# 51616/split-vae

Measured on AMD Instinct MI355X. Metric: images/sec training step, SPLIT-VAE CelebA-64 bs512, higher is better.
Workload: dtype f32 operands, f32 accumulate (exact-fp32 MFMA v_mfma_f32_16x16x4_f32): the reference's precision (vae/model.py:12); 1 GPU; SPLIT-VAE CelebA-64 64x64 beta=120 patch_size=8 latents=128+128 lr=1e-4, full train step (scramble+fwd+ELBO+bwd+Adam), per-GPU batch 512; global_batch=512, per_gpu_batch=512, parallelism=dp1, reconstructions=not stored (dead after the fused loss)

## Files before the change

split_vae_amd/csrc/kernels.h:

```cpp
#pragma once
#include <hip/hip_runtime.h>
#include <stdint.h>

#define SV_MAX_TAPS 81

struct TapGemmArgs {
  const void* A;
  const void* Wt;
  const float* bias;
  void* out;
  const void* mask;
  int M;
  int lOY, lOX;
  int OY, OX;
  int IH, IW, lda;
  int cl2;
  int P;
  int Ktot;
  int S, SX;
  int N;
  int OHF, OWF, OS, ooy, oox, ldo;
  int act, out_f32, splitk, ntaps;
  int ups;
  int d2s;
  int d2s_y;
  int clampin;
  int s2d3;
  const float* nll_img; void* nll_grad; float* nll_part; int nll_ch; float nll_gscale;
  int nll_noout;
  const float* fix;
  const float* fix2; int fix_nc, fix_pad;
  int cls_n;
  int accum;
  int adj;
  int8_t dy[SV_MAX_TAPS];
  int8_t dx[SV_MAX_TAPS];
};
int svk_tap_gemm(const TapGemmArgs& a, int dtype, int cfg, hipStream_t st);
#define SV_TAP_MAX_MULTI 4
struct TapGemmMulti {
  TapGemmArgs a[SV_TAP_MAX_MULTI];
  int zbase[SV_TAP_MAX_MULTI];
  int n;
};
int svk_tap_gemm_multi(const TapGemmArgs* a, int n, int dtype, int cfg, hipStream_t st);

struct TileConvArgs {
  const void* A; const void* Wt; const float* bias; void* out; const void* mask;
  int B, IH, IW, lda;
  int cl2, P, Ktot, S, SX;
  int lTW, lTH, lNB;
  int OY, OX, tilesX, tilesY, ntiles;
  int TIW, TIH, y_lo, x_lo;
  int PS;
  int plane_bytes;
  int nph, lnph;
  int xcd_chunk;
  int off_bytes, in_bytes;
  int buf_bytes;
  int wslots;
  int N, OHF, OWF, OS, ooy, oox, ldo, act, out_f32, ntaps;
  int dbg;
  int ups;
  int d2s;
  int cls_n;
  int d2s_y, clampin;
  int s2d3;
  int dma;
  const float* fix;
  const float* fix2; int fix_nc, fix_pad;
  const float* nll_img; void* nll_grad; float* nll_part; int nll_ch; float nll_gscale; int nll_noout;
  int8_t dy[SV_MAX_TAPS];
  int8_t dx[SV_MAX_TAPS];
};
#define SV_MAX_MULTI 8
#define SV_SHARED_STREAMS 3
hipStream_t sv_shared_stream(int k);
struct TileConvMulti { TileConvArgs a[SV_MAX_MULTI]; };
bool svk_tile_conv_plan(const TapGemmArgs& t, int dtype, int B, TileConvArgs* a, int* cfg_out);
int svk_tile_conv_multi(const TileConvArgs* a, int n, int dtype, int cfg, hipStream_t st);
int svk_conv_dispatch_multi(const TapGemmArgs* t, int n, int dtype, int tap_cfg, hipStream_t st);
int svk_tile_conv(const TileConvArgs& a, int dtype, int cfg, hipStream_t st);
int svk_row_conv_try(const TapGemmArgs* t, int n, int dtype, hipStream_t st);
bool svk_row_conv_supported(const TapGemmArgs* t, int n, int dtype);
int svk_conv_dispatch(const TapGemmArgs& t, int dtype, int tap_cfg, hipStream_t st);

struct WgradArgs {
  const void* A;
  const void* dY;
  float* dW;
  float* dbias;
  int M, lOY, lOX, OY, OX, IH, IW, lda, S, SX;
  int fold_kw, fold_c;
  int ldy, ycols;
  int cl2;
  int Cin_pad, Cin_real, N, Nrows;
  int ntaps, msplit;
  int ups;
  int clampin;
  int dy_s2d;
  int dy_os, dy_oy, dy_ox;
  int assign;
  int s2d3;
  float* ws;
  int64_t ws_bytes;
  hipEvent_t ev_mid[2];
  struct WgradReduceDesc* defer; int* n_defer;
  int8_t dy[SV_MAX_TAPS];
  int8_t dx[SV_MAX_TAPS];
};
int svk_wgrad(const WgradArgs& a, int dtype, int cfg, hipStream_t st);
#define SV_WGRAD_IM2COL_MAX_MULTI 4
struct WgradMulti {
  WgradArgs a[SV_WGRAD_IM2COL_MAX_MULTI];
  int zbase[SV_WGRAD_IM2COL_MAX_MULTI];
  int plain[SV_WGRAD_IM2COL_MAX_MULTI];
  int n;
};
int svk_wgrad_multi(const WgradArgs* a, int n, int dtype, int cfg, hipStream_t st);

struct WgradTileArgs {
  const void* A; const void* dY; float* dW; float* dbias;
  float* slab; float* ws; int64_t ws_bytes;
  float* bslab;
  struct WgradReduceDesc* defer; int* n_defer;
  int B, IH, IW, lda, cl2, S, SX, fold_kw, fold_c;
  int layer_id;
  int contig;
  int pairx;
  int lTW, lTH, lNB, OY, OX, tilesX, tilesY, ntiles;
  int TIW, TIH, y_lo, x_lo, PS;
  int ldy, YS, lycp;
// ... 126 lines not shown
```

split_vae_amd/csrc/lgvae_plan.hip:

```cpp
#include <string>
#include <algorithm>
#include <vector>
#include <map>
#include <stdio.h>
#include <stdlib.h>
#include <string.h>
#include "common.hip.h"
#include "kernels.h"
#include "conv_geom.h"

namespace {

__global__ void sv_plan_spin_kernel(long long ticks) {
  const long long t0 = wall_clock64();
  while (wall_clock64() - t0 < ticks) __builtin_amdgcn_s_sleep(32);
}
static void sv_plan_spin(hipStream_t st, int us) { hipLaunchKernelGGL(sv_plan_spin_kernel, dim3(1), dim3(64), 0, st, (long long)us * 100); }

struct Buf { std::string name; int64_t off, bytes; };

struct ParamInfo { std::string name; int64_t off; int ndim; int64_t shape[4]; int64_t count; };

static std::vector<ParamInfo> build_params(const sv_lgvae_desc* d) {
  std::vector<ParamInfo> v;
// ... 137 lines not shown
  int early_wait(hipStream_t st) {
    if (!early_pending) return SV_OK;
    early_pending = false;
    return hipStreamWaitEvent(st, ev_early_now, 0) == hipSuccess ? SV_OK : (int)hipGetLastError();
  }
  bool ensure_side() {
    if (nside) return true;
    {
      static const int want = getenv("SV_SIDE_STREAMS") ? atoi(getenv("SV_SIDE_STREAMS")) : 2;
      const int k = want < 1 ? 1 : want > SIDE_MAX - 1 ? SIDE_MAX - 1 : want;
      if (!ev_fork && hipEventCreateWithFlags(&ev_fork, hipEventDisableTiming) != hipSuccess) return false;
      for (int i = 0; i < k && i < SV_SHARED_STREAMS; ++i) {
        side[i] = sv_shared_stream(i);
        if (!side[i]) break;
        (void)hipEventCreateWithFlags(&ev_join[i], hipEventDisableTiming);
        ++nside;
      }
    }
    return nside > 0;
  }
  hipStream_t wgrad_stream(hipStream_t st) {
    side_slot = 0;
    if (!side_allowed()) return st;
    if (!ensure_side()) return st;
    const int use = side_use < nside ? side_use : nside;
    static const char* order = getenv("SV_SIDE_ORDER");
    int slot = side_next % use;
    if (order && order[0]) { const int c = order[side_count % (int)strlen(order)] - '0'; if (c >= 0 && c < use) slot = c; }
    ++side_count;
    hipEvent_t ef = fresh_event(ev_fork);
    if (hipEventRecord(ef, st) != hipSuccess || hipStreamWaitEvent(side[slot], ef, 0) != hipSuccess) return st;
    side_used[slot] = true;
    if (dbg_side_delay_us > 0 && side_count == 1) sv_plan_spin(side[slot], dbg_side_delay_us);
    side_next = slot + 1;
    side_slot = slot;
    side_pending = true;
    return side[slot];
  }
  int join_side(hipStream_t st) {
    const bool cap = graph_on || dyn;
    if (!side_pending && !(cap && side_used[0])) return SV_OK;
    side_pending = false;
    side_next = 0;
    side_count = 0;
    for (int i = 0; i < nside; ++i) {
      if (cap && !side_used[i]) continue;
      hipEvent_t ej = fresh_event(ev_join[i]);
      if (hipEventRecord(ej, side[i]) != hipSuccess || hipStreamWaitEvent(st, ej, 0) != hipSuccess) return (int)hipGetLastError();
    }
    return SV_OK;
  }
  int dbg_side_delay_us = 0;
  bool dbg_bucket_skip_side = false;
  hipEvent_t ev_bucket[3][1 + SIDE_MAX] = {};
  bool bucket_rec[3][1 + SIDE_MAX] = {};
  bool buckets_now = false;
  void clear_buckets() {
    for (auto& row : bucket_rec)
      for (auto& b : row) b = false;
  }
  int record_bucket(int k, hipStream_t st) {
    for (int i = 0; i <= SIDE_MAX; ++i) bucket_rec[k][i] = false;
    for (int i = 0; i <= nside; ++i) {
      hipStream_t s = i == 0 ? st : side[i - 1];
      if (i > 0 && !s) continue;
      if (!ev_bucket[k][i] && hipEventCreateWithFlags(&ev_bucket[k][i], hipEventDisableTiming) != hipSuccess) return (int)hipGetLastError();
      if (hipEventRecord(ev_bucket[k][i], s) != hipSuccess) return (int)hipGetLastError();
      bucket_rec[k][i] = true;
    }
    return SV_OK;
  }
  bool graph_on = false;
  const SvDynArgs* dyn = nullptr;
  struct HostState { bool gz_clean, dz_slabs, dz_valid, gz_zero_skipped, nll_fused; };
  HostState host_state() const { return {gz_clean, dz_slabs, dz_valid, gz_zero_skipped, nll_fused}; }
  void set_host_state(const HostState& h) { gz_clean = h.gz_clean; dz_slabs = h.dz_slabs; dz_valid = h.dz_valid; gz_zero_skipped = h.gz_zero_skipped; nll_fused = h.nll_fused; }
  uint64_t host_state_bits() const { return (uint64_t)gz_clean | (uint64_t)dz_slabs << 1 | (uint64_t)dz_valid << 2 | (uint64_t)gz_zero_skipped << 3 | (uint64_t)nll_fused << 4; }
  struct GraphEntry { hipGraphExec_t exec = nullptr; int seen = 0; HostState exit_state{}; };
  std::map<std::vector<uint64_t>, GraphEntry> graphs;
  bool prof_on;
  std::string prof_filter;
  std::vector<ProfEntry> prof;
  std::map<std::string, int> profidx;
  std::vector<ProfPending> pending;
  std::vector<hipEvent_t> event_pool;

  size_t esz() const { return d.dtype == SV_BF16 ? 2 : 4; }
  int ndec() const { return d.global_only ? 1 : 2; }
  int lc() const { return d.global_only ? d.global_latent : d.global_latent + d.local_latent; }
  int64_t add_buf(const std::string& n, int64_t bytes) {
    Buf b;
    b.name = n; b.off = ws_bytes; b.bytes = bytes;
    ws_bytes += (bytes + 255) / 256 * 256;
    bufidx[n] = (int)bufs.size();
    bufs.push_back(b);
    return b.off;
  }
  void* bp(const std::string& n) const {
    auto it = bufidx.find(n);
    return it == bufidx.end() ? nullptr : (void*)(ws + bufs[it->second].off);
  }
  int64_t bbytes(const std::string& n) const { return bufs[bufidx.at(n)].bytes; }
};

namespace {

// ... 1057 lines not shown
  build_buffers(p);
  *out = p;
  return SV_OK;
}

extern "C" void sv_lgvae_plan_destroy(sv_lgvae_plan* p) {
  if (!p) return;
  for (auto& pe : p->pending) { (void)hipEventDestroy(pe.a); (void)hipEventDestroy(pe.b); }
  for (auto e : p->event_pool) (void)hipEventDestroy(e);
  for (int i = 0; i < p->nside; ++i) {
    (void)hipStreamSynchronize(p->side[i]);
    (void)hipEventDestroy(p->ev_join[i]);
  }
  if (p->ev_fork) (void)hipEventDestroy(p->ev_fork);
  if (p->ev_early) (void)hipEventDestroy(p->ev_early);
  for (auto e : p->ev_cap)
    if (e) (void)hipEventDestroy(e);
  for (auto& row : p->ev_bucket)
    for (auto e : row)
      if (e) (void)hipEventDestroy(e);
  if (!p->graphs.empty()) (void)hipDeviceSynchronize();
  for (auto& kv : p->graphs)
    if (kv.second.exec) (void)hipGraphExecDestroy(kv.second.exec);
  delete p;
}

extern "C" int64_t sv_lgvae_workspace_bytes(const sv_lgvae_plan* p) { return p ? p->ws_bytes : -1; }

extern "C" int sv_lgvae_plan_bind(sv_lgvae_plan* p, void* workspace, int64_t bytes, void* stream) {
  if (!p || !workspace) return SV_E_BADARG;
  if (bytes < p->ws_bytes) return SV_E_WORKSPACE;
  if ((uintptr_t)workspace & 255) return SV_E_BADARG;
  p->ws = (char*)workspace;
  hipStream_t st = (hipStream_t)stream;
  hipError_t e = hipMemsetAsync(workspace, 0, (size_t)p->ws_bytes, st);
  if (e != hipSuccess) return (int)e;
  e = hipMemcpyAsync(p->bp("jobs"), p->jobs.data(), p->jobs.size() * sizeof(PrepJob), hipMemcpyHostToDevice, st);
  if (e != hipSuccess) return (int)e;
  e = hipStreamSynchronize(st);
  if (e != hipSuccess) return (int)e;
  p->bound = true;
  return SV_OK;
}

extern "C" int sv_lgvae_buffer(const sv_lgvae_plan* p, const char* name, int64_t* offset, int64_t* bytes) {
  if (!p || !name) return SV_E_BADARG;
  auto it = p->bufidx.find(name);
  if (it == p->bufidx.end()) return SV_E_BADARG;
  if (offset) *offset = p->bufs[it->second].off;
  if (bytes) *bytes = p->bufs[it->second].bytes;
  return SV_OK;
}

static int run_phases(sv_lgvae_plan* p, const sv_lgvae_step_args* s, hipStream_t st) {
  const int ph = s->phases;
  p->n_cap = 0;
  for (auto& u : p->side_used) u = false;
  {
    static const int forced = getenv("SV_SIDE_STREAMS") ? atoi(getenv("SV_SIDE_STREAMS")) : 0;
    const bool whole = (ph & SV_PHASE_ALL) == SV_PHASE_ALL;
    p->side_use = forced > 0 ? forced : (whole && p->ndec() * p->d.B >= 512) ? 2 : 1;
  }
  const bool zero_here = (ph & SV_PHASE_LOSS) && s->grads;
  hipStream_t early = ((ph & SV_PHASE_PREP) && (ph & SV_PHASE_FWD_ENCODERS)) ? p->early_stream(st) : nullptr;
  if (early && zero_here) {
    if (hipMemsetAsync(s->grads, 0, (size_t)p->nparams * 4, early) != hipSuccess) return (int)hipGetLastError();
  }
  if (ph & SV_PHASE_PREP) SV_TRY(phase_prep(p, s, st, early));
  if (early) SV_TRY(p->early_done(early));
  static const bool no_fused_nll = getenv("SV_NO_FUSED_NLL") != nullptr;
  static const bool no_fused_nll_f32 = getenv("SV_NO_FUSED_NLL_F32") != nullptr;
  const bool want_nll = !no_fused_nll && (ph & SV_PHASE_FWD_DECODERS) && (ph & SV_PHASE_LOSS) && s->grads && s->images6 &&
                        (p->d.dtype == SV_BF16 || !no_fused_nll_f32);
  if (!(ph & SV_PHASE_FORWARD)) p->nll_fused = false;
  if (ph & SV_PHASE_FORWARD) SV_TRY(phase_forward(p, s, ph & SV_PHASE_FWD_ENCODERS, ph & SV_PHASE_FWD_DECODERS, st, want_nll));
  if (ph & SV_PHASE_LOSS) {
    if (s->grads && !early) {
      Scope sc(p, st, "zero_grads", 0, (double)p->nparams * 4);
      if (hipMemsetAsync(s->grads, 0, (size_t)p->nparams * 4, st) != hipSuccess) return (int)hipGetLastError();
    }
    SV_TRY(phase_loss(p, s, s->grads != nullptr, st));
  }
  SV_TRY(p->early_wait(st));
  const bool buckets = (ph & SV_PHASE_BUCKET_EVENTS) && !p->graph_on && !p->dyn;
  if (ph & SV_PHASE_BACKWARD) p->clear_buckets();
  p->buckets_now = buckets;
  if (ph & SV_PHASE_BWD_DECODERS) {
    SV_TRY(phase_bwd_decoders(p, s, st));
    if (buckets) SV_TRY(p->record_bucket(0, st));
  }
  if (ph & (SV_PHASE_BWD_ENC_HEADS | SV_PHASE_BWD_ENC_CONVS))
    SV_TRY(phase_bwd_encoders(p, s, ph & SV_PHASE_BWD_ENC_HEADS, ph & SV_PHASE_BWD_ENC_CONVS, st, buckets));
  SV_TRY(p->join_side(st));
  if (p->n_pending) {
    Scope sc(p, st, "wgrad.all.reduce", 0, 0);
    const int np = p->n_pending;
    p->n_pending = 0;
    SV_TRY(svk_wgrad_reduce_all(p->red_pending, np, st));
  }
  if (ph & SV_PHASE_ADAM) {
    Scope sc(p, st, "adam_step", 0, (double)p->nparams * 28);
    SV_TRY(svk_adam_step(s->params, s->grads, s->adam_m, s->adam_v, p->nparams, s->lr, s->beta1, s->beta2,
                         s->adam_eps, s->t, s->grad_scale, p->dyn, st));
  }
  return SV_OK;
}

// ... 25 lines not shown
  const float alpha = (ph & SV_PHASE_ADAM) ? (float)svk_adam_alpha(s->lr, s->beta1, s->beta2, s->t) : 0.f;
  SV_TRY(svk_set_dyn((SvDynArgs*)p->bp("dyn"), s->seed, s->step, s->sample_offset, alpha, st));
  if (!e.exec) {
    hipGraph_t g = nullptr;
    if (hipStreamBeginCapture(st, hipStreamCaptureModeThreadLocal) != hipSuccess) return (int)hipGetLastError();
    p->dyn = (const SvDynArgs*)p->bp("dyn");
    const int rc = run_phases(p, s, st);
    p->dyn = nullptr;
    const hipError_t he = hipStreamEndCapture(st, &g);
    if (rc || he != hipSuccess || !g) {
      if (g) (void)hipGraphDestroy(g);
      return rc ? rc : (int)he;
    }
    const hipError_t hi = hipGraphInstantiate(&e.exec, g, nullptr, nullptr, 0);
    (void)hipGraphDestroy(g);
    if (hi != hipSuccess) { e.exec = nullptr; return (int)hi; }
    e.exit_state = p->host_state();
  } else {
    p->set_host_state(e.exit_state);
  }
  if (hipGraphLaunch(e.exec, st) != hipSuccess) return (int)hipGetLastError();
  return SV_OK;
}

extern "C" int sv_lgvae_graph_enable(sv_lgvae_plan* p, int32_t enable) {
  if (!p) return SV_E_BADARG;
  if (enable && p->d.global_only) return SV_E_UNSUPPORTED;
  p->graph_on = enable != 0;
  if (!enable) {
    for (auto& kv : p->graphs)
      if (kv.second.exec) (void)hipGraphExecDestroy(kv.second.exec);
    p->graphs.clear();
  }
  return SV_OK;
}

extern "C" int sv_lgvae_bucket_wait(sv_lgvae_plan* p, int32_t bucket, void* stream) {
  if (!p || bucket < 0 || bucket > 3) return SV_E_BADARG;
  int n = 0;
  for (int k = (bucket == 3 ? 1 : bucket); k <= (bucket == 3 ? 2 : bucket); ++k)
    for (int i = 0; i <= sv_lgvae_plan::SIDE_MAX; ++i)
      if (p->bucket_rec[k][i]) {
        if (p->dbg_bucket_skip_side && i > 0) continue;
        if (hipStreamWaitEvent((hipStream_t)stream, p->ev_bucket[k][i], 0) != hipSuccess) return (int)hipGetLastError();
        ++n;
      }
  return n ? SV_OK : SV_E_STATE;
}

extern "C" int sv_lgvae_plan_debug(sv_lgvae_plan* p, const char* key, int64_t value) {
  if (!p || !key) return SV_E_BADARG;
  if (!strcmp(key, "side_delay_us")) { if (value < 0 || value > 1000000) return SV_E_BADARG; p->dbg_side_delay_us = (int)value; return SV_OK; }
  if (!strcmp(key, "bucket_skip_side")) { p->dbg_bucket_skip_side = value != 0; return SV_OK; }
  return SV_E_BADARG;
}

extern "C" int sv_lgvae_graph_count(const sv_lgvae_plan* p) {
  if (!p) return SV_E_BADARG;
  int n = 0;
  for (auto& kv : p->graphs) n += kv.second.exec != nullptr;
  return n;
}

extern "C" int sv_lgvae_profile_enable(sv_lgvae_plan* p, int32_t enable) {
  if (!p) return SV_E_BADARG;
  p->prof_on = enable != 0;
  if (enable) {
    for (auto& pe : p->pending) { p->event_pool.push_back(pe.a); p->event_pool.push_back(pe.b); }
    p->pending.clear();
    p->prof.clear();
    p->profidx.clear();
  }
  return SV_OK;
}

extern "C" int sv_lgvae_profile_filter(sv_lgvae_plan* p, const char* name) {
  if (!p) return SV_E_BADARG;
  p->prof_filter = name ? name : "";
  return SV_OK;
}

extern "C" int sv_lgvae_profile_read(sv_lgvae_plan* p, int32_t max_entries, char names[][64], double* total_ms,
                                     int32_t* launches, double* flops_per_launch, double* bytes_per_launch) {
  if (!p) return SV_E_BADARG;
  for (auto& pe : p->pending) {
    (void)hipEventSynchronize(pe.b);
    float ms = 0.f;
    if (hipEventElapsedTime(&ms, pe.a, pe.b) == hipSuccess) {
      p->prof[pe.entry].total_ms += ms;
      p->prof[pe.entry].launches += 1;
    }
    p->event_pool.push_back(pe.a);
    p->event_pool.push_back(pe.b);
  }
  p->pending.clear();
  int n = (int)p->prof.size();
  if (n > max_entries) n = max_entries;
  for (int i = 0; i < n; ++i) {
    if (names) snprintf(names[i], 64, "%s", p->prof[i].name.c_str());
    if (total_ms) total_ms[i] = p->prof[i].total_ms;
    if (launches) launches[i] = p->prof[i].launches;
    if (flops_per_launch) flops_per_launch[i] = p->prof[i].flops;
    if (bytes_per_launch) bytes_per_launch[i] = p->prof[i].bytes;
  }
  return n;
}
// ... 19 lines not shown
```

split_vae_amd/csrc/tile_conv.hip:

```cpp
#include "common.hip.h"
#include "kernels.h"
#include "tile_stage.hip.h"
#include "dlogistic.hip.h"
#include <stdio.h>
#include <stdlib.h>
#include <string.h>

#ifndef SV_TC_PPS16
#define SV_TC_PPS16 16
#endif
#ifndef SV_TC_PPS32
#define SV_TC_PPS32 8
#endif
#ifndef SV_TC_PPS64
#define SV_TC_PPS64 8
#endif
static __host__ __device__ constexpr int tile_pps(int BN, int YR = 0) {
  return YR ? (BN == 16 || YR == 5 ? YR * 4 : 8) : BN == 16 ? SV_TC_PPS16 : BN == 32 ? SV_TC_PPS32 : BN == 64 ? SV_TC_PPS64 : 8;
}

template <int PPS>
__device__ __forceinline__ int wpiece(int q, int n) {
  if constexpr (PPS % 8 == 0) return q ^ (n & 7);
  else return (q & ~7) == (PPS & ~7) ? (q & ~3) | ((q & 3) ^ (n & 3)) : q ^ (n & 7);
}

template <typename T> struct MmaOpT;
template <> struct MmaOpT<bf16_t> {
  static __device__ __forceinline__ void run(const uint4& a, const uint4& b, f32x4& c) {
    c = __builtin_amdgcn_mfma_f32_16x16x32_bf16(__builtin_bit_cast(bf16x8, a), __builtin_bit_cast(bf16x8, b), c, 0, 0, 0);
  }
};
template <> struct MmaOpT<float> {
  static __device__ __forceinline__ void run(const uint4& a, const uint4& b, f32x4& c) {
    const float4 af = __builtin_bit_cast(float4, a), bf = __builtin_bit_cast(float4, b);
    c = __builtin_amdgcn_mfma_f32_16x16x4f32(af.x, bf.x, c, 0, 0, 0);
    c = __builtin_amdgcn_mfma_f32_16x16x4f32(af.y, bf.y, c, 0, 0, 0);
    c = __builtin_amdgcn_mfma_f32_16x16x4f32(af.z, bf.z, c, 0, 0, 0);
    c = __builtin_amdgcn_mfma_f32_16x16x4f32(af.w, bf.w, c, 0, 0, 0);
  }
};

static constexpr int tile_min_waves(int BN, int NW, int YR, bool WR = false) { return (YR || WR) && NW == 4 ? (BN == 64 ? 3 : 4) : 1; }
template <typename T, int BN, int MF, int NW, int YR, bool WR, bool FX = false>
__global__ __launch_bounds__(64 * NW, tile_min_waves(BN, NW, YR, WR)) void tile_conv_kernel(const TileConvMulti mg) {
  const TileConvArgs& g = mg.a[blockIdx.z];
  if (SV_DBG(g.dbg) & 32) return;
  constexpr int NT = 64 * NW, WM = 16 * MF, BM = NW * WM, NF = BN / 16;
  constexpr int PPS = tile_pps(BN, YR), RB = PPS * 16;
  constexpr int RPP = NT / PPS;
  constexpr int BRN = (BN + RPP - 1) / RPP;
  constexpr int EPP = ElemTraits<T>::EPP;
  extern __shared__ __attribute__((aligned(16))) char smem[];
  char* sB = smem;
  int* sOff = (int*)(smem + g.wslots * BN * RB);
  char* sIn = smem + g.wslots * BN * RB + g.off_bytes;

  const int tid = threadIdx.x, lane = tid & 63, wave = tid >> 6;
  int t = blockIdx.x;
  if (g.xcd_chunk) {
    const int remapped = (t & 7) * g.xcd_chunk + (t >> 3);
    t = remapped < g.ntiles && (g.ntiles & 7) == 0 ? remapped : t;
  }
  const int tx0 = (t % g.tilesX) << g.lTW; t /= g.tilesX;
  const int ty0 = (t % g.tilesY) << g.lTH; t /= g.tilesY;
  const int b0 = t << g.lNB;
  const int n0 = blockIdx.y * BN;
  const int TW = 1 << g.lTW, TH = 1 << g.lTH, NB = 1 << g.lNB;
  const int cpp = 1 << g.cl2;

  const T* __restrict__ Wb = (const T*)g.Wt;
  const int nph = g.nph, lcH = g.cl2 - g.lnph;
  const int gP = g.P >> g.lnph, gKtot = g.Ktot, gdbg = SV_DBG(g.dbg);
  const int pp = tid % PPS, r0 = tid / PPS;
  int ph = 0;
  uint4 rbA[BRN];
  auto load_b = [&](int ks, uint4 (&rb)[BRN]) {
    const int pl = ks * PPS + pp;
    const bool pv = pl < gP;
    const int p = ((pl >> lcH) << g.cl2) + (ph << lcH) + (pl & ((1 << lcH) - 1));
#pragma unroll
    for (int i = 0; i < BRN; ++i) {
      const int n = r0 + RPP * i;
      rb[i] = (pv && n < BN && r0 < RPP) ? *(const uint4*)(Wb + (int64_t)(n0 + n) * gKtot + (int64_t)p * EPP) : make_uint4(0, 0, 0, 0);
    }
  };
  auto write_b = [&](int slot, const uint4 (&rb)[BRN]) {
#pragma unroll
    for (int i = 0; i < BRN; ++i) {
      const int n = r0 + RPP * i;
      if (n < BN && r0 < RPP) *(uint4*)(sB + slot * (BN * RB) + n * RB + (wpiece<PPS>(pp, n) << 4)) = rb[i];
    }
  };
  const int nk = (gdbg & 2) ? 0 : (gP + PPS - 1) / PPS;
  constexpr int WRMAX = 6;
  constexpr bool wres = WR && YR == 0;
  uint4 rbw[wres ? WRMAX - 1 : 1][BRN];
  load_b(0, rbA);
  if constexpr (wres) {
#pragma unroll
    for (int ks = 1; ks < WRMAX; ++ks) load_b(ks, rbw[ks - 1]);
  }

  const int nkp = (gP + PPS - 1) / PPS * PPS;
  for (int p = tid; p < nkp; p += NT) {
    int off = 0;
    if (p < gP) {
      const int tap = p >> lcH, c = p & ((1 << lcH) - 1);
      const int tp = ((int)g.dy[tap] - g.y_lo) * g.TIW + ((int)g.dx[tap] - g.x_lo);
      off = g.plane_bytes ? tp * 32 + (c >> 1) * g.plane_bytes + (c & 1) * 16 : tp * g.PS + c * 16;
    }
    sOff[p] = off;
  }
  auto stage = [&](int phase) {
    if (SV_DBG(g.dbg) & 1) return;
    const TileStageGeom sg = {g.B, g.IH, g.IW, g.lda, lcH, g.TIW, g.TIH, g.PS, NB, g.plane_bytes};
    const int iy_base = ty0 * g.S + g.y_lo, ix_base = tx0 * g.SX + g.x_lo;
    const T* Ap = (const T*)g.A + ((phase << lcH) * EPP);
    if constexpr (sizeof(T) == 4) {
      if (g.s2d3) { stage_tile_s2d3<NT>((const float*)g.A, sg, b0, iy_base, ix_base, sIn, tid); return; }
    }
    if (g.ups) stage_tile_upsampled<T, NT>(Ap, sg, b0, iy_base, ix_base, sIn, tid);
    else if (sizeof(T) == 4 && g.dma) {
      const int wv = __builtin_amdgcn_readfirstlane(wave);
      if (g.clampin) stage_tile_plain_dma<T, NW, true>(Ap, sg, b0, iy_base, ix_base, sIn, lane, wv);
// ... 39 lines not shown
  };
  constexpr int SPG = YR ? YR * 4 / PPS : 1, TPS = PPS / 4;
  const int rowpitch = g.TIW * g.PS;
  for (ph = 0; ph < nph; ++ph) {
    if (ph) {
      load_b(0, rbA);
      stage(ph);
    }
    write_b(0, rbA);
    if constexpr (wres) {
#pragma unroll
      for (int ks = 1; ks < WRMAX; ++ks)
        if (ks < nk) write_b(ks, rbw[ks - 1]);
    }
    __syncthreads();
    if constexpr (YR > 0) {
      for (int gq = 0; gq * SPG < nk; ++gq) {
        uint4 aw[MF + YR - 1];
        const char* wp = sIn + lbase[0] + sOff[gq * (YR * 4) + lg];
#pragma unroll
        for (int iy = 0; iy < MF + YR - 1; ++iy) aw[iy] = *(const uint4*)(wp + iy * rowpitch);
#pragma unroll
        for (int sg = 0; sg < SPG; ++sg) {
          const int ks = gq * SPG + sg;
          const bool more = ks + 1 < nk;
          if (more) load_b(ks + 1, rbA);
          const char* cB = sB + (ks & 1) * (BN * RB);
#pragma unroll
          for (int kk = 0; kk < TPS; ++kk) {
            uint4 bfr[NF];
#pragma unroll
            for (int j = 0; j < NF; ++j) {
              const int n = j * 16 + lr;
              bfr[j] = *(const uint4*)(cB + n * RB + (wpiece<PPS>(kk * 4 + lg, n) << 4));
            }
#pragma unroll
            for (int i = 0; i < MF; ++i)
#pragma unroll
              for (int j = 0; j < NF; ++j) MmaOpT<T>::run(bfr[j], aw[i + sg * TPS + kk], acc[i][j]);
          }
          if (more) write_b((ks & 1) ^ 1, rbA);
          __syncthreads();
        }
      }
    } else if constexpr (wres) {
      for (int ks = 0; ks < nk; ++ks) compute(ks, ks);
      __syncthreads();
    } else
    for (int ks = 0; ks < nk; ++ks) {
      const bool more = ks + 1 < nk && !(gdbg & 8);
      if (more) load_b(ks + 1, rbA);
      compute(ks, ks & 1);
      if (more) write_b((ks & 1) ^ 1, rbA);
      if (!(gdbg & 16)) __syncthreads();
    }
    if (nk == 0) __syncthreads();
  }

  const int oesz = g.out_f32 ? 4 : (int)sizeof(T);
  const int Nst = (!g.d2s && !g.cls_n && (g.N & 7)) ? min(g.ldo, (g.N + 7) & ~7) : g.N;
  const int ncols = min(BN, Nst - n0);
  const int rowb = g.d2s ? (g.d2s_y ? 4 : 2) * g.d2s * 4 : ncols * oesz;
  const int srow = ((rowb + 15) & ~15) + 16;
  char* sC = smem;
  float bv[NF][4];
#pragma unroll
  for (int j = 0; j < NF; ++j)
#pragma unroll
    for (int e = 0; e < 4; ++e) {
      const int nl = j * 16 + lg * 4 + e;
      const int bi = g.d2s ? (nl & 7) : n0 + nl;
      bv[j][e] = (g.bias && nl < ncols && n0 + nl < g.N && (!g.d2s || bi < g.d2s)) ? g.bias[bi] : 0.f;
    }
  const bool relu = g.act == SV_ACT_RELU;
#pragma unroll
  for (int i = 0; i < MF; ++i) {
    const int r = wave * WM + i * 16 + lr;
    constexpr bool FIXC = FX || sizeof(T) == 4;
    const float *frp = nullptr, *fcp = nullptr;
    if (FIXC && g.fix_nc) {
      const int tx = r & (TW - 1), ty = (r >> g.lTW) & (TH - 1), bl = r >> (g.lTW + g.lTH);
      const int b = b0 + bl, R = (ty0 + ty) * g.OS + g.ooy, Cc = (tx0 + tx) * g.OS + g.oox, nbot = g.fix_nc - g.fix_pad;
      const int rc = R < g.fix_pad ? R : R >= g.OHF - nbot ? g.fix_pad + R - (g.OHF - nbot) : -1;
      const int cc = Cc < g.fix_pad ? Cc : Cc >= g.OWF - nbot ? g.fix_pad + Cc - (g.OWF - nbot) : -1;
      if (b < g.B && rc >= 0) frp = g.fix + (((int64_t)b * g.fix_nc + rc) * g.OWF + Cc) * g.N + n0;
      if (b < g.B && cc >= 0) fcp = g.fix2 + (((int64_t)b * g.OHF + R) * g.fix_nc + cc) * g.N + n0;
    }
#pragma unroll
    for (int j = 0; j < NF; ++j) {
      const int nl = j * 16 + lg * 4;
      if (nl >= ncols) continue;
      float v[4];
      float fv[4] = {0.f, 0.f, 0.f, 0.f};
      if constexpr (FIXC) {
        float4 fr = make_float4(0.f, 0.f, 0.f, 0.f), fc = fr;
        if (frp) fr = *(const float4*)(frp + nl);
        if (fcp) fc = *(const float4*)(fcp + nl);
        fv[0] = fr.x + fc.x; fv[1] = fr.y + fc.y; fv[2] = fr.z + fc.z; fv[3] = fr.w + fc.w;
      }
#pragma unroll
      for (int e = 0; e < 4; ++e) {
        v[e] = acc[i][j][e] + bv[j][e];
        if (FIXC && g.fix_nc) v[e] += fv[e];
        if (relu) v[e] = fmaxf(v[e], 0.f);
      }
      if (g.d2s) {
        const int px = nl >> 3, c0 = nl & 7;
#pragma unroll
        for (int e = 0; e < 4; ++e)
// ... 93 lines not shown
        fr[u] = fc[u] = make_float4(0.f, 0.f, 0.f, 0.f);
        if (g.fix && lo[u] >= 0) {
          const int rc = R < 2 ? R : R >= g.OHF - 3 ? R - (g.OHF - 5) : -1;
          const int cg = ox == 0 ? 0 : ox == g.OX - 2 ? 1 : ox == g.OX - 1 ? 2 : -1;
          const float* fb = g.fix + (int64_t)b * (5 * g.OWF + 6 * g.OHF) * C;
          if (rc >= 0) fr[u] = *(const float4*)(fb + ((int64_t)rc * g.OWF + ox * 2) * C + cs * 4);
          if (cg >= 0) fc[u] = *(const float4*)(fb + (int64_t)5 * g.OWF * C + ((int64_t)R * 3 + cg) * 2 * C + cs * 4);
        }
      }
#pragma unroll
      for (int u = 0; u < 4; ++u) {
        if (lo[u] < 0) continue;
        float4 v = *(const float4*)(sC + lo[u]);
        v.x = (v.x + fr[u].x) + fc[u].x; v.y = (v.y + fr[u].y) + fc[u].y;
        v.z = (v.z + fr[u].z) + fc[u].z; v.w = (v.w + fr[u].w) + fc[u].w;
        *(float4*)((char*)g.out + ob[u]) = v;
      }
    }
    return;
  }
  for (int q = tid; q < BM * ppr_o; q += NT) {
    const int r = q / ppr_o, c = q - r * ppr_o;
    const int tx = r & (TW - 1), ty = (r >> g.lTW) & (TH - 1), bl = r >> (g.lTW + g.lTH);
    const int b = b0 + bl, oy = ty0 + ty, ox = tx0 + tx;
    if (b >= g.B || oy >= g.OY || ox >= g.OX) continue;
    int64_t ob;
    if (g.cls_n) {
      const int n = n0 + c * (psz / oesz), cls = n / g.cls_n, ch = n - cls * g.cls_n;
      const int64_t pix = ((int64_t)b * g.OHF + oy * g.OS + (cls >> 1)) * g.OWF + ox * g.OS + (cls & 1);
      ob = (pix * g.ldo + ch) * oesz;
    } else {
      const int64_t pix = ((int64_t)b * g.OHF + oy * g.OS + g.ooy) * g.OWF + ox * (g.d2s ? 2 : g.OS) + g.oox;
      ob = (pix * g.ldo + n0) * oesz + c * psz;
    }
    if (psz == 16) {
      uint4 v = *(const uint4*)(sC + r * srow + c * 16);
      if (g.mask) {
        const uint4 mv = *(const uint4*)((const char*)g.mask + ob);
        T ve[EPP], me[EPP];
        *(uint4*)ve = v; *(uint4*)me = mv;
#pragma unroll
        for (int e = 0; e < EPP; ++e) ve[e] = to_f32(me[e]) > 0.f ? ve[e] : from_f32<T>(0.f);
        v = *(uint4*)ve;
      }
      *(uint4*)((char*)g.out + ob) = v;
    } else {
      *(uint2*)((char*)g.out + ob) = *(const uint2*)(sC + r * srow + c * 8);
    }
  }
}

static inline size_t tile_lds_bytes(int BN, int BM, const TileConvArgs& a, size_t esz, int YR = 0) {
  size_t lds = (size_t)a.wslots * BN * tile_pps(BN, YR) * 16 + a.off_bytes + a.in_bytes;
  const size_t epi = (size_t)BM * (((BN * (a.out_f32 ? 4 : esz) + 15) & ~(size_t)15) + 16);
  return lds < epi ? epi : lds;
}

template <typename T, int BN, int MF, int NW = 4, int YR = 0, bool WR = false, bool FX = false>
static int launch_tile(const TileConvArgs* a, int n, hipStream_t st) {
  const int Npad = round_up(a[0].N, BN);
  dim3 grid(a[0].ntiles, Npad / BN, n), block(64 * NW);
  size_t lds = 0;
  TileConvMulti m;
  for (int i = 0; i < n; ++i) {
    m.a[i] = a[i];
    const size_t l = tile_lds_bytes(BN, NW * 16 * MF, a[i], sizeof(T), YR);
    if (l > lds) lds = l;
  }
  sv_ensure_dynamic_lds((const void*)tile_conv_kernel<T, BN, MF, NW, YR, WR, FX>, lds);
  hipLaunchKernelGGL((tile_conv_kernel<T, BN, MF, NW, YR, WR, FX>), grid, block, lds, st, m);
  SV_LAUNCH_CHECK();
  return SV_OK;
}

static bool tile_conv_plan_impl(const TapGemmArgs& t, int dtype, int B, TileConvArgs* a, int* cfg_out, bool narrow, int64_t* lds_out);
bool svk_tile_conv_plan(const TapGemmArgs& t, int dtype, int B, TileConvArgs* a, int* cfg_out) {
  int64_t lds = 0;
  if (!tile_conv_plan_impl(t, dtype, B, a, cfg_out, false, &lds)) return false;
  static const bool no_narrow = getenv("SV_TC_NO_LDS_NARROW") != nullptr;
  if (!no_narrow && dtype == SV_F32 && t.N % 128 == 0 && !t.cls_n && lds > 78 * 1024) {
    TileConvArgs b;
    int c = 0;
    int64_t l2 = 0;
    if (tile_conv_plan_impl(t, dtype, B, &b, &c, true, &l2) && l2 <= 78 * 1024) { *a = b; *cfg_out = c; }
  }
  return true;
}
static bool tile_conv_plan_impl(const TapGemmArgs& t, int dtype, int B, TileConvArgs* a, int* cfg_out, bool narrow, int64_t* lds_out) {
  if (t.splitk != 1 || t.accum) return false;
  if (t.lOY < 0 || t.lOX < 0 || t.S > 2) return false;
  const int OY = 1 << t.lOY, OX = 1 << t.lOX;
  if (t.ups && t.S != 1) return false;
  if (t.d2s && ((t.N != 16 && !(t.N == 32 && t.d2s_y)) || !t.out_f32)) return false;
  if (t.d2s_y && (!t.d2s || t.N != 32 || ((2 * t.d2s * 4) & 7))) return false;
  if (t.clampin && (t.ups || t.S != 1)) return false;
  if (t.s2d3 && (dtype != SV_F32 || t.S != 1 || t.SX != 1 || t.ups || t.clampin || t.cl2 != 2)) return false;
  if (t.fix_nc && !t.d2s_y && ((dtype != SV_F32 && t.S != 2) || !t.fix || !t.fix2 || (t.N & 15) || t.out_f32)) return false;
  if (t.nll_part && (!t.d2s_y || t.d2s != 6 || OY * OX < 256 || !t.nll_img || !t.nll_grad)) return false;
  if (t.cls_n && (t.OS != 2 || t.N != 4 * t.cls_n || (t.cls_n & 7) || t.out_f32 || t.bias)) return false;
  if (OY * OX < 16) return false;
  if (!t.d2s && !t.cls_n) {
    const int oe = t.out_f32 ? 4 : (dtype == SV_BF16 ? 2 : 4);
    const int nst = (t.N & 7) ? (t.ldo < ((t.N + 7) & ~7) ? t.ldo : ((t.N + 7) & ~7)) : t.N;
    if ((nst * oe) & 7) return false;
  }
  const int esz = dtype == SV_BF16 ? 2 : 4, epp = 16 / esz;
  const int cin = (1 << t.cl2) * epp;
// ... 61 lines not shown
    if (MF == 4 && BN == 32 && dtype == SV_F32 && !t.nll_part && wgs < small32_wgs) continue;
    int lnph = 0, PS = 0, plane_bytes = 0;
    int64_t in_bytes = 0;
    bool planar = false;
    for (;; ++lnph) {
      if (yr) lnph = t.cl2 - 2;
      const int pbh = pb >> lnph;
      PS = layout(pbh, &planar);
      plane_bytes = planar ? NB * TIH * TIW * 32 : 0;
      in_bytes = planar ? (int64_t)plane_bytes * (pbh / 32) : (int64_t)NB * TIH * TIW * PS;
      static const int ph_kb = getenv("SV_TC_PH_KB") ? atoi(getenv("SV_TC_PH_KB")) : 53;
      static const bool s2_phases = getenv("SV_TC_NPH_NO_S2") == nullptr;
      static const int ph_wgs = getenv("SV_TC_PH_WGS") ? atoi(getenv("SV_TC_PH_WGS")) : 256;
      const int64_t tot = in_bytes + 2 * BN * tile_pps(BN) * 16 + off_bytes;
      if (yr || t.s2d3 || !((2 << lnph) <= nph_max && (pbh >> 1) >= 32 && (planar || s2_phases) &&
                            ((wgs >= ph_wgs && tot > ph_kb * 1024) || tot > 150 * 1024))) break;
    }
    static const bool wres_on = getenv("SV_TC_NO_WRES") == nullptr;
    const int nks = (int)(((t.P >> lnph) + tile_pps(BN) - 1) / tile_pps(BN));
    const int wslots = (wres_on && !yr && dtype == SV_BF16 && BN == 32 && MF == 4 && t.S == 1 && lnph == 0 && nks > 2 && nks <= 6 && nks * BN * tile_pps(BN) * 16 <= 24 * 1024) ? nks : 2;
    const int64_t lds = (int64_t)wslots * BN * tile_pps(BN, yr) * 16 + off_bytes + in_bytes;
    if (lds > 78 * 1024 && MF == 4 && BN >= 64) continue;
    static const bool s2_mf4 = getenv("SV_TC_S2_MF4") != nullptr;
    if (lds > 78 * 1024 && MF == 4 && t.S == 2 && t.fix_nc && !s2_mf4) continue;
    *lds_out = lds;
    if (lds > 150 * 1024) {
      if (MF == 4) continue;
      if (getenv("SV_TC_VERBOSE")) fprintf(stderr, "tile_conv plan: REFUSED (LDS %lld) N=%d cin=%d S=%d ntaps=%d\n", (long long)lds, t.N, cin, t.S, t.ntaps);
      return false;
    }
    memset(a, 0, sizeof(*a));
    a->A = t.A; a->Wt = t.Wt; a->bias = t.bias; a->out = t.out; a->mask = t.mask;
    a->B = B; a->IH = t.IH; a->IW = t.IW; a->lda = t.lda;
    a->cl2 = t.cl2; a->P = t.P; a->Ktot = t.Ktot; a->S = t.S; a->SX = t.SX; a->d2s = t.d2s; a->cls_n = t.cls_n; a->d2s_y = t.d2s_y; a->clampin = t.clampin; a->fix = t.fix;
    a->fix2 = t.fix2; a->fix_nc = t.d2s_y ? 0 : t.fix_nc; a->fix_pad = t.fix_pad; a->s2d3 = t.s2d3;
    a->nll_img = t.nll_img; a->nll_grad = t.nll_grad; a->nll_part = t.nll_part; a->nll_ch = t.nll_ch; a->nll_gscale = t.nll_gscale; a->nll_noout = t.nll_noout;
    a->lTW = lTW; a->lTH = lTH; a->lNB = lNB;
    a->OY = OY; a->OX = OX;
    a->tilesX = OX / TW; a->tilesY = OY / TH;
    a->ntiles = a->tilesX * a->tilesY * ((B + NB - 1) / NB);
    a->TIW = TIW; a->TIH = TIH; a->y_lo = y_lo; a->x_lo = x_lo; a->PS = PS; a->plane_bytes = plane_bytes;
    a->nph = 1 << lnph; a->lnph = lnph; a->wslots = wslots;
    {
      static const bool no_dma = getenv("SV_TC_NO_DMA") != nullptr;
      a->dma = (!no_dma && dtype == SV_F32 && !t.ups && !t.s2d3 && (planar || PS == (pb >> lnph))) ? 1 : 0;
    }
    if (getenv("SV_TC_VERBOSE")) fprintf(stderr, "tile_conv plan: yr=%d wslots=%d N=%d BN=%d MF=%d cin=%d pb=%d planar=%d nph=%d tile=%dx%dx%d PS=%d in_bytes=%lld lds=%lld ntiles=%d S=%d SX=%d\n", yr, wslots, t.N, BN, MF, cin, pb, (int)planar, 1 << lnph, NB, TIH, TIW, PS, (long long)in_bytes, (long long)lds, a->ntiles, t.S, t.SX);
    {
      static const bool xcd = getenv("SV_TC_NO_XCD") == nullptr;
      a->xcd_chunk = (xcd && a->ntiles >= 64 && (a->ntiles & 7) == 0) ? a->ntiles / 8 : 0;
    }
    a->off_bytes = off_bytes; a->in_bytes = (int)in_bytes;
    a->N = t.N; a->OHF = t.OHF; a->OWF = t.OWF; a->OS = t.OS; a->ooy = t.ooy; a->oox = t.oox; a->ldo = t.ldo;
    a->act = t.act; a->out_f32 = t.out_f32; a->ntaps = t.ntaps; a->ups = t.ups;
    memcpy(a->dy, t.dy, sizeof(a->dy));
    memcpy(a->dx, t.dx, sizeof(a->dx));
    *cfg_out = cfgN * 2 + (MF == 4 ? 0 : 1) + (yr == 4 ? 32 : yr == 6 ? 64 : yr == 5 ? 96 : 0) + (wslots > 2 ? 128 : 0);
    static const char* nw8 = getenv("SV_TC_NW8");
    if (MF == 4 && dtype == SV_BF16 && nw8 && strchr(nw8, BN == 16 ? 'a' : BN == 32 ? 'b' : BN == 64 ? 'c' : 'd')) *cfg_out = 16 + cfgN;
    return true;
  }
  return false;
}

int svk_tile_conv_multi(const TileConvArgs* a, int n, int dtype, int cfg, hipStream_t st) {
  if (n < 1 || n > SV_MAX_MULTI) return SV_E_BADARG;
  if (dtype == SV_BF16 && a[0].fix_nc) {
    switch (cfg) {
      case 2: return launch_tile<bf16_t, 64, 4, 4, 0, false, true>(a, n, st);
      case 3: return launch_tile<bf16_t, 64, 2, 4, 0, false, true>(a, n, st);
      case 4: return launch_tile<bf16_t, 32, 4, 4, 0, false, true>(a, n, st);
      case 5: return launch_tile<bf16_t, 32, 2, 4, 0, false, true>(a, n, st);
    }
    return SV_E_UNSUPPORTED;
  }
  if (dtype == SV_BF16) {
    switch (cfg) {
      case 0: return launch_tile<bf16_t, 128, 4>(a, n, st);
      case 1: return launch_tile<bf16_t, 128, 2>(a, n, st);
      case 2: return launch_tile<bf16_t, 64, 4>(a, n, st);
      case 3: return launch_tile<bf16_t, 64, 2>(a, n, st);
      case 4: return launch_tile<bf16_t, 32, 4>(a, n, st);
      case 5: return launch_tile<bf16_t, 32, 2>(a, n, st);
      case 7: return launch_tile<bf16_t, 16, 2>(a, n, st);
      case 6: return launch_tile<bf16_t, 16, 4>(a, n, st);
      case 128 + 4: return launch_tile<bf16_t, 32, 4, 4, 0, true>(a, n, st);
      case 32 + 2: return launch_tile<bf16_t, 64, 4, 4, 4>(a, n, st);
      case 32 + 4: return launch_tile<bf16_t, 32, 4, 4, 4>(a, n, st);
      case 32 + 6: return launch_tile<bf16_t, 16, 4, 4, 4>(a, n, st);
      case 96 + 4: return launch_tile<bf16_t, 32, 4, 4, 5>(a, n, st);
      case 64 + 2: return launch_tile<bf16_t, 64, 4, 4, 6>(a, n, st);
      case 64 + 4: return launch_tile<bf16_t, 32, 4, 4, 6>(a, n, st);
      case 64 + 6: return launch_tile<bf16_t, 16, 4, 4, 6>(a, n, st);
      case 16: return launch_tile<bf16_t, 128, 2, 8>(a, n, st);
      case 17: return launch_tile<bf16_t, 64, 2, 8>(a, n, st);
      case 18: return launch_tile<bf16_t, 32, 2, 8>(a, n, st);
      case 19: return launch_tile<bf16_t, 16, 2, 8>(a, n, st);
    }
  } else if (dtype == SV_F32) {
    switch (cfg) {
      case 1: return launch_tile<float, 128, 2>(a, n, st);
      case 2: return launch_tile<float, 64, 4>(a, n, st);
      case 3: return launch_tile<float, 64, 2>(a, n, st);
      case 4: return launch_tile<float, 32, 4>(a, n, st);
      case 5: return launch_tile<float, 32, 2>(a, n, st);
      case 7: return launch_tile<float, 16, 2>(a, n, st);
      case 6: return launch_tile<float, 16, 4>(a, n, st);
    }
  }
  return SV_E_BADARG;
}

int svk_tile_conv(const TileConvArgs& a, int dtype, int cfg, hipStream_t st) { return svk_tile_conv_multi(&a, 1, dtype, cfg, st); }

static const char* tile_form(const TapGemmArgs& t) { return t.s2d3 ? "tile_s2d3" : (t.d2s && !t.d2s_y) ? "tile_packx" : "tile"; }

// ... 63 lines not shown
```

Before: 56110 images/s.

## Store fp32 tile-conv accumulators directly to global, skipping LDS epilogue

For fp32 tile convolutions, the epilogue now writes each wave's MFMA accumulator fragments straight to global memory as float4 stores. It applies bias, the fix border terms, ReLU and the mask in registers, and drops the final barrier and the LDS staging buffer. The smaller LDS need is paired with a higher launch-bounds minimum-wave hint for some BN/MF configs to raise occupancy. The trade-off is less coalesced global writes, since each lane stores 16-byte pieces scattered across rows. A debug key restores the old LDS epilogue.

```diff
diff --git a/split_vae_amd/csrc/kernels.h b/split_vae_amd/csrc/kernels.h
--- a/split_vae_amd/csrc/kernels.h
+++ b/split_vae_amd/csrc/kernels.h
@@ -67,6 +67,7 @@
   int d2s_y, clampin;
   int s2d3;
   int dma;
+  int epi_direct;
   const float* fix;
   const float* fix2; int fix_nc, fix_pad;
   const float* nll_img; void* nll_grad; float* nll_part; int nll_ch; float nll_gscale; int nll_noout;
@@ -78,6 +79,7 @@
 hipStream_t sv_shared_stream(int k);
 struct TileConvMulti { TileConvArgs a[SV_MAX_MULTI]; };
 bool svk_tile_conv_plan(const TapGemmArgs& t, int dtype, int B, TileConvArgs* a, int* cfg_out);
+extern thread_local bool sv_tile_lds_epilogue;
 int svk_tile_conv_multi(const TileConvArgs* a, int n, int dtype, int cfg, hipStream_t st);
 int svk_conv_dispatch_multi(const TapGemmArgs* t, int n, int dtype, int tap_cfg, hipStream_t st);
 int svk_tile_conv(const TileConvArgs& a, int dtype, int cfg, hipStream_t st);
diff --git a/split_vae_amd/csrc/lgvae_plan.hip b/split_vae_amd/csrc/lgvae_plan.hip
--- a/split_vae_amd/csrc/lgvae_plan.hip
+++ b/split_vae_amd/csrc/lgvae_plan.hip
@@ -213,6 +213,7 @@
   }
   int dbg_side_delay_us = 0;
   bool dbg_bucket_skip_side = false;
+  bool dbg_tile_lds_epi = false;
   hipEvent_t ev_bucket[3][1 + SIDE_MAX] = {};
   bool bucket_rec[3][1 + SIDE_MAX] = {};
   bool buckets_now = false;
@@ -1376,7 +1377,15 @@
   return SV_OK;
 }
 
+static int run_phases_body(sv_lgvae_plan* p, const sv_lgvae_step_args* s, hipStream_t st);
 static int run_phases(sv_lgvae_plan* p, const sv_lgvae_step_args* s, hipStream_t st) {
+  const bool keep = sv_tile_lds_epilogue;
+  sv_tile_lds_epilogue = p->dbg_tile_lds_epi;
+  const int rc = run_phases_body(p, s, st);
+  sv_tile_lds_epilogue = keep;
+  return rc;
+}
+static int run_phases_body(sv_lgvae_plan* p, const sv_lgvae_step_args* s, hipStream_t st) {
   const int ph = s->phases;
   p->n_cap = 0;
   for (auto& u : p->side_used) u = false;
@@ -1508,6 +1517,7 @@
   if (!p || !key) return SV_E_BADARG;
   if (!strcmp(key, "side_delay_us")) { if (value < 0 || value > 1000000) return SV_E_BADARG; p->dbg_side_delay_us = (int)value; return SV_OK; }
   if (!strcmp(key, "bucket_skip_side")) { p->dbg_bucket_skip_side = value != 0; return SV_OK; }
+  if (!strcmp(key, "tile_lds_epilogue")) { p->dbg_tile_lds_epi = value != 0; return SV_OK; }
   return SV_E_BADARG;
 }
 
diff --git a/split_vae_amd/csrc/tile_conv.hip b/split_vae_amd/csrc/tile_conv.hip
--- a/split_vae_amd/csrc/tile_conv.hip
+++ b/split_vae_amd/csrc/tile_conv.hip
@@ -41,9 +41,11 @@
   }
 };
 
-static constexpr int tile_min_waves(int BN, int NW, int YR, bool WR = false) { return (YR || WR) && NW == 4 ? (BN == 64 ? 3 : 4) : 1; }
+static constexpr int tile_min_waves(int BN, int MF, int NW, int YR, bool WR = false, int esz = 2) {
+  return (YR || WR) && NW == 4 ? (BN == 64 ? 3 : 4) : (esz == 4 && NW == 4 && !YR && !WR && (BN == 32 || (BN == 64 && MF == 2))) ? 4 : 1;
+}
 template <typename T, int BN, int MF, int NW, int YR, bool WR, bool FX = false>
-__global__ __launch_bounds__(64 * NW, tile_min_waves(BN, NW, YR, WR)) void tile_conv_kernel(const TileConvMulti mg) {
+__global__ __launch_bounds__(64 * NW, tile_min_waves(BN, MF, NW, YR, WR, (int)sizeof(T))) void tile_conv_kernel(const TileConvMulti mg) {
   const TileConvArgs& g = mg.a[blockIdx.z];
   if (SV_DBG(g.dbg) & 32) return;
   constexpr int NT = 64 * NW, WM = 16 * MF, BM = NW * WM, NF = BN / 16;
@@ -71,6 +73,7 @@
 
   const T* __restrict__ Wb = (const T*)g.Wt;
   const int nph = g.nph, lcH = g.cl2 - g.lnph;
+  const bool epi_direct = sizeof(T) == 4 && g.epi_direct;
   const int gP = g.P >> g.lnph, gKtot = g.Ktot, gdbg = SV_DBG(g.dbg);
   const int pp = tid % PPS, r0 = tid / PPS;
   int ph = 0;
@@ -216,9 +219,69 @@
       if (more) load_b(ks + 1, rbA);
       compute(ks, ks & 1);
       if (more) write_b((ks & 1) ^ 1, rbA);
-      if (!(gdbg & 16)) __syncthreads();
+      if (!(gdbg & 16) && !(epi_direct && ks + 1 == nk && ph + 1 == nph)) __syncthreads();
     }
     if (nk == 0) __syncthreads();
+  }
+
+  if constexpr (sizeof(T) == 4) {
+    if (epi_direct) {
+      const int Nst = (!g.cls_n && (g.N & 7)) ? min(g.ldo, (g.N + 7) & ~7) : g.N;
+      const int ncols = min(BN, Nst - n0);
+      float bv[NF][4];
+#pragma unroll
+      for (int j = 0; j < NF; ++j)
+#pragma unroll
+        for (int e = 0; e < 4; ++e) {
+          const int nl = j * 16 + lg * 4 + e;
+          bv[j][e] = (g.bias && nl < ncols && n0 + nl < g.N) ? g.bias[n0 + nl] : 0.f;
+        }
+      const bool relu = g.act == SV_ACT_RELU, store = !(SV_DBG(g.dbg) & 4);
+#pragma unroll
+      for (int i = 0; i < MF; ++i) {
+        const int r = wave * WM + i * 16 + lr;
+        const int tx = r & (TW - 1), ty = (r >> g.lTW) & (TH - 1), bl = r >> (g.lTW + g.lTH);
+        const int b = b0 + bl, oy = ty0 + ty, ox = tx0 + tx;
+        const float *frp = nullptr, *fcp = nullptr;
+        if (g.fix_nc) {
+          const int R = oy * g.OS + g.ooy, Cc = ox * g.OS + g.oox, nbot = g.fix_nc - g.fix_pad;
+          const int rc = R < g.fix_pad ? R : R >= g.OHF - nbot ? g.fix_pad + R - (g.OHF - nbot) : -1;
+          const int cc = Cc < g.fix_pad ? Cc : Cc >= g.OWF - nbot ? g.fix_pad + Cc - (g.OWF - nbot) : -1;
+          if (b < g.B && rc >= 0) frp = g.fix + (((int64_t)b * g.fix_nc + rc) * g.OWF + Cc) * g.N + n0;
+          if (b < g.B && cc >= 0) fcp = g.fix2 + (((int64_t)b * g.OHF + R) * g.fix_nc + cc) * g.N + n0;
+        }
+        const bool live = b < g.B && oy < g.OY && ox < g.OX && store;
+        const int64_t pix = ((int64_t)b * g.OHF + oy * g.OS + g.ooy) * g.OWF + ox * g.OS + g.oox;
+#pragma unroll
+        for (int j = 0; j < NF; ++j) {
+          const int nl = j * 16 + lg * 4;
+          if (nl >= ncols) continue;
+          float4 fr = make_float4(0.f, 0.f, 0.f, 0.f), fc = fr;
+          if (frp) fr = *(const float4*)(frp + nl);
+          if (fcp) fc = *(const float4*)(fcp + nl);
+          const float fv[4] = {fr.x + fc.x, fr.y + fc.y, fr.z + fc.z, fr.w + fc.w};
+          float v[4];
+#pragma unroll
+          for (int e = 0; e < 4; ++e) {
+            v[e] = acc[i][j][e] + bv[j][e];
+            if (g.fix_nc) v[e] += fv[e];
+            if (relu) v[e] = fmaxf(v[e], 0.f);
+          }
+          if (!live) continue;
+          int64_t ob;
+          if (g.cls_n) {
+            const int n = n0 + nl, cls = n / g.cls_n, ch = n - cls * g.cls_n;
+            ob = (((int64_t)b * g.OHF + oy * g.OS + (cls >> 1)) * g.OWF + ox * g.OS + (cls & 1)) * g.ldo + ch;
+          } else ob = pix * g.ldo + n0 + nl;
+          if (g.mask) {
+            const float4 m = *(const float4*)((const float*)g.mask + ob);
+            v[0] = m.x > 0.f ? v[0] : 0.f; v[1] = m.y > 0.f ? v[1] : 0.f; v[2] = m.z > 0.f ? v[2] : 0.f; v[3] = m.w > 0.f ? v[3] : 0.f;
+          }
+          *(float4*)((float*)g.out + ob) = make_float4(v[0], v[1], v[2], v[3]);
+        }
+      }
+      return;
+    }
   }
 
   const int oesz = g.out_f32 ? 4 : (int)sizeof(T);
@@ -418,7 +481,7 @@
 
 static inline size_t tile_lds_bytes(int BN, int BM, const TileConvArgs& a, size_t esz, int YR = 0) {
   size_t lds = (size_t)a.wslots * BN * tile_pps(BN, YR) * 16 + a.off_bytes + a.in_bytes;
-  const size_t epi = (size_t)BM * (((BN * (a.out_f32 ? 4 : esz) + 15) & ~(size_t)15) + 16);
+  const size_t epi = a.epi_direct ? 0 : (size_t)BM * (((BN * (a.out_f32 ? 4 : esz) + 15) & ~(size_t)15) + 16);
   return lds < epi ? epi : lds;
 }
 
@@ -586,6 +649,10 @@
     }
     a->off_bytes = off_bytes; a->in_bytes = (int)in_bytes;
     a->N = t.N; a->OHF = t.OHF; a->OWF = t.OWF; a->OS = t.OS; a->ooy = t.ooy; a->oox = t.oox; a->ldo = t.ldo;
+    {
+      const int nst = (!t.cls_n && (t.N & 7)) ? (t.ldo < ((t.N + 7) & ~7) ? t.ldo : ((t.N + 7) & ~7)) : t.N;
+      a->epi_direct = (dtype == SV_F32 && !t.d2s && !t.nll_part && (nst & 3) == 0 && (t.ldo & 3) == 0 && !sv_tile_lds_epilogue) ? 1 : 0;
+    }
     a->act = t.act; a->out_f32 = t.out_f32; a->ntaps = t.ntaps; a->ups = t.ups;
     memcpy(a->dy, t.dy, sizeof(a->dy));
     memcpy(a->dx, t.dx, sizeof(a->dx));
@@ -596,6 +663,8 @@
   }
   return false;
 }
+
+thread_local bool sv_tile_lds_epilogue = false;
 
 int svk_tile_conv_multi(const TileConvArgs* a, int n, int dtype, int cfg, hipStream_t st) {
   if (n < 1 || n > SV_MAX_MULTI) return SV_E_BADARG;
```

Measured after the change: 56270 images/s (median of 6 runs). No clear change (+0.3%).
